# threewisemonkeys-as/torched_impala

Hardware: NVIDIA H100
Metric: learner steps/sec on synthetic (T=20,B=4096) trajectories (higher is better)
Workload: dtype f32

## Files before the change

torched_impala_b200/_cabi.py:

```python
from __future__ import annotations

import ctypes as C
import os

_HERE = os.path.dirname(os.path.abspath(__file__))
LIB_PATH = os.path.join(_HERE, "lib", "libimpala_b200.so")

MODE_REFERENCE = 0
MODE_PAPER = 1
MODES = {"reference": MODE_REFERENCE, "paper": MODE_PAPER}

OBS_F32 = 0
OBS_U8 = 1
OBS_DTYPES = {"float32": OBS_F32, "uint8": OBS_U8}

OPT_ADAM = 0
OPT_RMSPROP = 1
OPT_RULES = {"adam": OPT_ADAM, "rmsprop": OPT_RMSPROP}
POPART_STATS = 5
REWARD_CLIP_ABS_ONE = 1
REWARD_CLIP_SOFT_ASYMMETRIC = 2
REWARD_CLIPS = {"abs_one": REWARD_CLIP_ABS_ONE, "soft_asymmetric": REWARD_CLIP_SOFT_ASYMMETRIC}


def obs_dtype_code(obs_dtype: str) -> int:
    if obs_dtype not in OBS_DTYPES:
        raise ValueError(f"obs_dtype must be one of {sorted(OBS_DTYPES)}, got {obs_dtype!r}")
    return OBS_DTYPES[obs_dtype]


def reward_clip_code(reward_clip) -> int:
    if reward_clip is None:
        return 0
    if not isinstance(reward_clip, str) or reward_clip not in REWARD_CLIPS:
        raise ValueError(f"reward_clip must be None or one of {sorted(REWARD_CLIPS)}, got {reward_clip!r}")
    return REWARD_CLIPS[reward_clip]

ACT_CATEGORICAL = 0
ACT_GAUSSIAN = 1
ACT_DISTS = {"categorical": ACT_CATEGORICAL, "gaussian": ACT_GAUSSIAN}
MAX_GAUSSIAN_DIMS = 16


def act_kind_code(action_dist: str) -> int:
    if not isinstance(action_dist, str) or action_dist not in ACT_DISTS:
        raise ValueError(f"action_dist must be one of {sorted(ACT_DISTS)}, got {action_dist!r}")
    return ACT_DISTS[action_dist]


_ERRORS = {-1: "IMPALA_ERR_BAD_ARG", -2: "IMPALA_ERR_UNSUPPORTED_SHAPE",
           -3: "IMPALA_ERR_WORKSPACE_TOO_SMALL"}

_p = C.c_void_p
_i = C.c_int
_i64 = C.c_int64
_f = C.c_float

SIGNATURES = {
    "impala_abi_version": (_i, []),
# ... 113 lines not shown
```

torched_impala_b200/build.py:

```python
from __future__ import annotations

import concurrent.futures as cf
import os
import shutil
import subprocess
import sys

HERE = os.path.dirname(os.path.abspath(__file__))
CSRC = os.path.join(HERE, "csrc")
_LIB_DIR = os.environ.get("IMPALA_LIB_DIR", os.path.join(HERE, "lib"))
OBJ = os.path.join(_LIB_DIR, "obj")
LIB = os.path.join(_LIB_DIR, "libimpala_b200.so")

ARCH = ["-gencode", "arch=compute_90a,code=sm_90a"]
COMMON = ["-O3", "-lineinfo", "-std=c++17", "-Xcompiler", "-fPIC", "-Xptxas", "-v"]
MLP_WIDTHS = (8, 24, 32, 64, 128)


def _nvcc() -> str:
    for cand in (shutil.which("nvcc"), "/usr/local/cuda/bin/nvcc"):
        if cand and os.path.exists(cand):
            return cand
    raise RuntimeError("nvcc not found: the CUDA extension cannot be built")


def _units():
    units = [("mlp", "mlp.cu", []), ("vtrace_loss", "vtrace_loss.cu", []),
             ("vtrace_loss_rclip", "vtrace_loss_rclip.cu", []), ("vtrace_loss_gauss", "vtrace_loss_gauss.cu", []),
             ("optim", "optim.cu", []), ("abi", "abi.cu", []),
             ("mlp_fwd_tc", "mlp_fwd_tc.cu", []), ("mlp_bwd_tc", "mlp_bwd_tc.cu", []),
             ("loss_terms", "loss_terms.cu", []), ("mlp_obs_tc", "mlp_obs_tc.cu", []),
             ("obs_frames", "obs_frames.cu", []), ("batch_compose", "batch_compose.cu", [])]
    for op in MLP_WIDTHS:
        for bwd in (0, 1):
            units.append((f"mlp_inst_op{op}_{'bwd' if bwd else 'fwd'}", "mlp_inst.cu",
                          [f"-DIMPALA_OP={op}", f"-DIMPALA_BWD={bwd}"]))
    return units


def _newest_source_mtime() -> float:
    paths = [os.path.join(CSRC, f) for f in os.listdir(CSRC)]
    paths.append(os.path.join(HERE, "..", "include", "impala_b200.h"))
    paths.append(os.path.abspath(__file__))
    return max(os.path.getmtime(p) for p in paths)


def _compile(nvcc, name, src, defs, stamp):
    obj = os.path.join(OBJ, name + ".o")
    log = os.path.join(OBJ, name + ".ptxas.log")
    if os.path.exists(obj) and os.path.getmtime(obj) >= stamp:
        return name, 0, "cached"
    cmd = [nvcc, *ARCH, *COMMON, *defs, "-c", os.path.join(CSRC, src), "-o", obj]
    res = subprocess.run(cmd, capture_output=True, text=True)
    with open(log, "w") as f:
        f.write(res.stderr)
    return name, res.returncode, res.stderr if res.returncode else "built"


def build(verbose: bool = False, jobs: int | None = None) -> str:
    nvcc = _nvcc()
    os.makedirs(OBJ, exist_ok=True)
    stamp = _newest_source_mtime()
    units = _units()
    jobs = jobs or min(len(units), os.cpu_count() or 4)
    with cf.ThreadPoolExecutor(jobs) as ex:
        results = list(ex.map(lambda u: _compile(nvcc, *u, stamp), units))
    for name, rc, msg in results:
        if rc:
            raise RuntimeError(f"nvcc failed on {name}:\n{msg}")
        if verbose:
            print(f"[build] {name}: {msg}")
    objs = [os.path.join(OBJ, u[0] + ".o") for u in units]
    if (not os.path.exists(LIB)) or any(os.path.getmtime(o) > os.path.getmtime(LIB) for o in objs):
        cmd = [nvcc, *ARCH, "-shared", "-cudart", "static", "-o", LIB, *objs]
        res = subprocess.run(cmd, capture_output=True, text=True)
        if res.returncode:
            raise RuntimeError(f"link failed:\n{res.stderr}")
        if verbose:
            print(f"[build] linked {LIB}")
    return LIB


if __name__ == "__main__":
    print(build(verbose=True))
    sys.exit(0)
```

torched_impala_b200/csrc/mlp_bwd_tc.cu:

```cuda
#include "mlp_kernels.cuh"
#include "tc_common.cuh"

namespace {

constexpr int kRowsT = 64;
constexpr int kWG = 2;
constexpr int kThreads = kWG * 128;
constexpr int kWarps = kThreads / 32;
constexpr int kHB = 64 * kWG;
constexpr int kXAtomBytes = kRowsT * 128;

struct BwdTcArgs {
    const float* x;
    const float* params;
    const float* dout;
    float* ws;
    double* grad;
    unsigned int* ctl;
    int M, O, H, N2, num_tiles;
    MlpLayout lay;
};

struct BwdTcSplitArgs : BwdTcArgs {
    const float* dout_b;
    int M_a;
};
template <bool SPLIT>
using BwdArgs = std::conditional_t<SPLIT, BwdTcSplitArgs, BwdTcArgs>;

template <bool SPLIT>
__device__ __forceinline__ float load_dz(const BwdArgs<SPLIT>& a, int row, int n0, int n) {
    if constexpr (SPLIT) return split_dz(a.dout, a.dout_b, a.M_a, a.N2, row, n0 + n);
    else return __ldg(a.dout + (size_t)row * a.N2 + n0 + n);
}

__host__ __device__ constexpr size_t bwd_smem_bytes(int ka, int np) {
    return 1024 + (size_t)2 * ka * kHB * 128 + (size_t)2 * ka * (ka == 4 ? 32 : kRowsT) * 128 +
           (size_t)2 * ((ka == 4 ? 32 : kRowsT) / 32) * 32 * ka * 128 +
           (size_t)(ka == 4 ? 32 : kRowsT) * (np > 4 ? np + 4 : np) * sizeof(float) +
           (np > 4 ? (size_t)kHB * (np + 4) * sizeof(float) + 8 * 32 * sizeof(float) : 4 * sizeof(float));
}

__device__ __forceinline__ float f4(const float4& v, int e) { return e == 0 ? v.x : e == 1 ? v.y : e == 2 ? v.z : v.w; }

template <int NP, int KA, bool SPLIT = false>
__device__ __forceinline__ uint8_t* bwd_tc_body(const BwdArgs<SPLIT>& a, const int cta, const int ncta) {
    extern __shared__ uint8_t smem_raw[];
    uint8_t* smem = smem_raw + ((1024u - (tc::smem_u32(smem_raw) & 1023u)) & 1023u);
    constexpr bool X4 = KA == 4;
    constexpr bool L2S = NP > 4;
    constexpr int RT = X4 ? 32 : kRowsT;
    constexpr int NB = RT / 32;
    constexpr int FA = X4 ? 2 : KA;
// ... 438 lines not shown
        for (int sgm = 0; sgm < 4; ++sgm)
            for (int64_t p = lo4[sgm] + tid; p < hi4[sgm]; p += kThreads) wsb[p] = 0.f;
    }

    constexpr int kLd = kRowsT * 8 / 128;
    const int rr = 16 * warp + (lane & 15);
    float4 v[kLd];
    float z[NP];
    auto load = [&](int tile) {
#pragma unroll
        for (int k = 0; k < kLd; ++k) {
            const int c = 2 * k + (lane >> 4), row = tile * kRowsT + rr;
            v[k] = make_float4(0.f, 0.f, 0.f, 0.f);
            if (k < ksteps && tile < a.num_tiles && row < a.M && c < ochunks)
                v[k] = __ldg(reinterpret_cast<const float4*>(a.x + (size_t)row * O) + c);
        }
        const int row = tile * kRowsT + lt;
#pragma unroll
        for (int n = 0; n < NP; ++n)
            z[n] = (lt < kRowsT && tile < a.num_tiles && row < a.M && n < a.N2) ? load_dz<SPLIT>(a, row, 0, n) : 0.f;
    };
    float gb2[NP];
#pragma unroll
    for (int n = 0; n < NP; ++n) gb2[n] = 0.f;

    pdl_wait();
    const int j0 = 64 * grp + 16 * warp + g, j1 = j0 + 8;
    uint32_t wh[4][4], wl[4][4];
#pragma unroll
    for (int kk = 0; kk < 4; ++kk)
#pragma unroll
        for (int i = 0; i < 4; ++i) {
            const int f = 8 * kk + q + 4 * (i >> 1);
            float hi, lo;
            tc::split_tf32(f < O ? __ldg(W1 + (size_t)(i & 1 ? j1 : j0) * O + f) : 0.f, hi, lo);
            wh[kk][i] = __float_as_uint(hi), wl[kk][i] = __float_as_uint(lo);
        }
    const float bj0 = __ldg(b1 + j0), bj1 = __ldg(b1 + j1);
    float w2r0[NP], w2r1[NP], gw0[NP], gw1[NP], gb10 = 0.f, gb11 = 0.f;
#pragma unroll
    for (int n = 0; n < NP; ++n) {
        w2r0[n] = n < a.N2 ? __ldg(W2 + (size_t)n * H + j0) : 0.f;
        w2r1[n] = n < a.N2 ? __ldg(W2 + (size_t)n * H + j1) : 0.f;
        gw0[n] = gw1[n] = 0.f;
    }
    float acc_hh[16], acc_c[16];
#pragma unroll
    for (int i = 0; i < 16; ++i) acc_hh[i] = acc_c[i] = 0.f;
    tc::fence_acc(acc_hh), tc::fence_acc(acc_c);
    const uint64_t dx_hi = tc::smem_desc_k_sw128(x_hi, 0), dx_lo = tc::smem_desc_k_sw128(x_lo, 0);
    const uint64_t dxt_hi = tc::smem_desc_k_sw128(xt_hi, 0), dxt_lo = tc::smem_desc_k_sw128(xt_lo, 0);

    const int bar = 1 + wg, tstride = 2 * cpg;
    load(r + cpg * wg);
    for (int tile = r + cpg * wg; tile < a.num_tiles; tile += tstride) {
        tc::named_bar(bar, 128);
#pragma unroll
        for (int k = 0; k < kLd; ++k) {
            if (k >= ksteps) continue;
            const int c = 2 * k + (lane >> 4);
            float4 hi, lo;
            tc::split4(v[k], hi, lo);
            const uint32_t off = tc::sw128_offset(rr, c);
            *reinterpret_cast<float4*>(x_hi + off) = hi;
            *reinterpret_cast<float4*>(x_lo + off) = lo;
            const int r32 = rr & 31, pos = (r32 & ~7) + ((r32 & 7) >> 1) + 4 * (r32 & 1);
#pragma unroll
            for (int e = 0; e < 4; ++e) {
                const int f = 4 * c + e;
                const uint32_t toff = (rr >> 5) * (32 * 128) + (f >> 3) * 1024 + (f & 7) * 128 +
                                      (((pos >> 2) ^ (f & 7)) << 4) + (pos & 3) * 4;
                *reinterpret_cast<float*>(xt_hi + toff) = f4(hi, e);
                *reinterpret_cast<float*>(xt_lo + toff) = f4(lo, e);
            }
        }
        if (lt < kRowsT) {
#pragma unroll
            for (int n = 0; n < NP; ++n) dzs[lt * NP + n] = z[n], gb2[n] += z[n];
        }
        tc::fence_proxy_async();
        tc::named_bar(bar, 128);
        load(tile + tstride);

        uint64_t bx_hi = dx_hi, bx_lo = dx_lo;
        asm volatile("" : "+l"(bx_hi), "+l"(bx_lo));
        float d[32];
#pragma unroll
        for (int i = 0; i < 32; ++i) d[i] = 0.f;
        tc::fence_acc(d);
        tc::wgmma_fence();
#pragma unroll
        for (int kk = 0; kk < 4; ++kk) {
            if (kk < ksteps) {
                const uint32_t xo = (kk * 32) >> 4;
                tc::wgmma_n64_rs(d, wl[kk], bx_hi + xo, kk > 0);
                tc::wgmma_n64_rs(d, wh[kk], bx_lo + xo, true);
            }
        }
#pragma unroll
        for (int kk = 0; kk < 4; ++kk) {
            if (kk < ksteps) tc::wgmma_n64_rs(d, wh[kk], bx_hi + ((kk * 32) >> 4), true);
        }
        tc::wgmma_commit();
        tc::wgmma_wait<0>();
        tc::fence_acc(d);

#pragma unroll
        for (int i = 0; i < 8; ++i) {
#pragma unroll
            for (int e = 0; e < 2; ++e) {
                const int m = 8 * i + 2 * q + e;
                float dz[NP];
                if constexpr (NP == 4) {
                    const float4 t = *reinterpret_cast<const float4*>(dzs + 4 * m);
                    dz[0] = t.x, dz[1] = t.y, dz[2] = t.z, dz[3] = t.w;
                } else {
                    dz[0] = dzs[m];
                }
                const float pre0 = d[4 * i + e] + bj0, pre1 = d[4 * i + 2 + e] + bj1;
                const float h0 = fmaxf(pre0, 0.f), h1 = fmaxf(pre1, 0.f);
                float dh0 = dz[0] * w2r0[0], dh1 = dz[0] * w2r1[0];
#pragma unroll
                for (int n = 1; n < NP; ++n) dh0 = fmaf(dz[n], w2r0[n], dh0), dh1 = fmaf(dz[n], w2r1[n], dh1);
#pragma unroll
                for (int n = 0; n < NP; ++n) gw0[n] = fmaf(dz[n], h0, gw0[n]), gw1[n] = fmaf(dz[n], h1, gw1[n]);
                const float dp0 = pre0 > 0.f ? dh0 : 0.f, dp1 = pre1 > 0.f ? dh1 : 0.f;
                gb10 += dp0, gb11 += dp1;
                d[4 * i + e] = dp0, d[4 * i + 2 + e] = dp1;
            }
        }

        uint32_t lo[32];
#pragma unroll
        for (int i = 0; i < 32; ++i) {
            const float hi = __uint_as_float(__float_as_uint(d[i]) & 0xffffe000u);
            lo[i] = __float_as_uint(d[i] - hi);
            d[i] = hi;
        }
        uint64_t bxt_hi = dxt_hi, bxt_lo = dxt_lo;
        asm volatile("" : "+l"(bxt_hi), "+l"(bxt_lo));
        tc::wgmma_fence();
#pragma unroll
        for (int kk = 0; kk < 8; ++kk) {
            const uint32_t al[4] = {lo[4 * kk], lo[4 * kk + 2], lo[4 * kk + 1], lo[4 * kk + 3]};
            const uint32_t ah[4] = {__float_as_uint(d[4 * kk]), __float_as_uint(d[4 * kk + 2]),
                                    __float_as_uint(d[4 * kk + 1]), __float_as_uint(d[4 * kk + 3])};
            const uint32_t xo = ((kk >> 2) * 32 * 128 + (kk & 3) * 32) >> 4;
            tc::wgmma_n32_rs(acc_c, al, bxt_hi + xo, true);
            tc::wgmma_n32_rs(acc_c, ah, bxt_lo + xo, true);
            tc::wgmma_n32_rs(acc_hh, ah, bxt_hi + xo, true);
        }
        tc::wgmma_commit();
        tc::wgmma_wait<0>();
        tc::fence_acc(d);
#pragma unroll
        for (int i = 0; i < 32; ++i) asm volatile("" : "+r"(lo[i])::"memory");
        tc::fence_acc(acc_hh), tc::fence_acc(acc_c);
    }

#pragma unroll
    for (int s = 1; s <= 2; s <<= 1) {
        gb10 += __shfl_xor_sync(IMPALA_FULL_MASK, gb10, s);
        gb11 += __shfl_xor_sync(IMPALA_FULL_MASK, gb11, s);
#pragma unroll
        for (int n = 0; n < NP; ++n) {
            gw0[n] += __shfl_xor_sync(IMPALA_FULL_MASK, gw0[n], s);
            gw1[n] += __shfl_xor_sync(IMPALA_FULL_MASK, gw1[n], s);
        }
    }
    float gwt[16];
#pragma unroll
    for (int i = 0; i < 16; ++i) gwt[i] = acc_hh[i] + acc_c[i];
#pragma unroll
    for (int n = 0; n < NP; ++n) {
#pragma unroll
        for (int off = 16; off > 0; off >>= 1) gb2[n] += __shfl_xor_sync(IMPALA_FULL_MASK, gb2[n], off);
    }
    if (lt < kRowsT && lane == 0) {
#pragma unroll
        for (int n = 0; n < NP; ++n) gb2x[(2 * wg + warp) * 4 + n] = gb2[n];
    }
    float* xch = reinterpret_cast<float*>(smem + kStageBytes);
    __syncthreads();
    if (wg == 1) {
#pragma unroll
        for (int i = 0; i < 16; ++i) xch[i * 128 + lt] = gwt[i];
        xch[16 * 128 + lt] = gb10, xch[17 * 128 + lt] = gb11;
#pragma unroll
        for (int n = 0; n < NP; ++n) xch[(18 + n) * 128 + lt] = gw0[n], xch[(18 + NP + n) * 128 + lt] = gw1[n];
    }
    __syncthreads();
    if (wg == 0) {
#pragma unroll
        for (int i = 0; i < 16; ++i) gwt[i] += xch[i * 128 + lt];
        gb10 += xch[16 * 128 + lt], gb11 += xch[17 * 128 + lt];
#pragma unroll
        for (int n = 0; n < NP; ++n) gw0[n] += xch[(18 + n) * 128 + lt], gw1[n] += xch[(18 + NP + n) * 128 + lt];
        if (q == 0) {
            wsb[a.lay.ob1 + j0] = gb10;
            wsb[a.lay.ob1 + j1] = gb11;
#pragma unroll
            for (int n = 0; n < NP; ++n)
                if (n < a.N2) wsb[a.lay.oW2 + (size_t)n * H + j0] = gw0[n], wsb[a.lay.oW2 + (size_t)n * H + j1] = gw1[n];
        }
#pragma unroll
        for (int i = 0; i < 4; ++i) {
            const int f = 8 * i + 2 * q;
            if (f < O) {
                *reinterpret_cast<float2*>(wsb + a.lay.oW1 + (size_t)j0 * O + f) = make_float2(gwt[4 * i], gwt[4 * i + 1]);
                *reinterpret_cast<float2*>(wsb + a.lay.oW1 + (size_t)j1 * O + f) = make_float2(gwt[4 * i + 2], gwt[4 * i + 3]);
            }
        }
        if (grp == 0 && tid == 0) {
#pragma unroll
            for (int n = 0; n < NP; ++n)
                if (n < a.N2) wsb[a.lay.ob2 + n] = (gb2x[n] + gb2x[4 + n]) + (gb2x[8 + n] + gb2x[12 + n]);
        }
    }
    __threadfence();
    __syncthreads();
    return smem;
}

__device__ __forceinline__ void grid_arrive_and_wait(unsigned int* ctl) {
    if (threadIdx.x == 0) {
        atomicAdd(ctl, 1u);
        const long long t0 = clock64();
        unsigned int seen;
        do {
            asm volatile("ld.acquire.gpu.global.u32 %0, [%1];" : "=r"(seen) : "l"(ctl) : "memory");
            if (seen != gridDim.x && clock64() - t0 > (1ll << 32)) __trap();
        } while (seen != gridDim.x);
    }
    __syncthreads();
}

__device__ __forceinline__ void grid_depart(unsigned int* ctl) {
    if (threadIdx.x == 0 && atomicAdd(ctl + 1, 1u) == gridDim.x - 1) {
        ctl[0] = 0u;
        ctl[1] = 0u;
    }
}

__device__ __forceinline__ void reduce_rows(const BwdTcArgs& a, const int nparts, const int first,
                                            const int stride, double* s_red, const PushArgs* push = nullptr,
                                            const int64_t push_off = 0) {
    const int warp = threadIdx.x >> 5, lane = threadIdx.x & 31;
    const int64_t total = a.lay.total;
    const int nchunks = (int)((total + 63) >> 6);
    for (int c = first; c < nchunks; c += stride) {
        const int64_t e0 = (int64_t)c * 64 + 2 * lane;
        double sx = 0.0, sy = 0.0;
        if (e0 < total) {
            const float* col = a.ws + e0;
            int p = warp;
            for (; p + 3 * kWarps < nparts; p += 4 * kWarps) {
                const float2 v0 = __ldcg(reinterpret_cast<const float2*>(col + (size_t)p * total));
                const float2 v1 = __ldcg(reinterpret_cast<const float2*>(col + (size_t)(p + kWarps) * total));
                const float2 v2 = __ldcg(reinterpret_cast<const float2*>(col + (size_t)(p + 2 * kWarps) * total));
                const float2 v3 = __ldcg(reinterpret_cast<const float2*>(col + (size_t)(p + 3 * kWarps) * total));
                sx += v0.x, sy += v0.y, sx += v1.x, sy += v1.y;
                sx += v2.x, sy += v2.y, sx += v3.x, sy += v3.y;
            }
            for (; p < nparts; p += kWarps) {
                const float2 v0 = __ldcg(reinterpret_cast<const float2*>(col + (size_t)p * total));
                sx += v0.x, sy += v0.y;
            }
        }
        s_red[warp * 64 + 2 * lane] = sx;
        s_red[warp * 64 + 2 * lane + 1] = sy;
        __syncthreads();
        if (push) {
            if (warp < push->world) {
// ... 126 lines not shown
    if (cpg < 1) return IMPALA_ERR_UNSUPPORTED_SHAPE;
    e = dout_b ? impala_launch_ex(mlp_bwd_tc_split_kernel, nblk * cpg, kThreads, smem, st, true, true, a)
               : impala_launch_ex(kernel, nblk * cpg, kThreads, smem, st, true, true, static_cast<const BwdTcArgs&>(a));
    if (e != cudaSuccess) return (int)e;
    return impala_launch_status();
}

int impala_mlp_bwd_tc_pair(const float* x, const float* params_pi, const float* params_vf,
                           const float* dlogits, const float* dv, float* ws_pi, float* ws_vf,
                           double* grad_pi, double* grad_vf, unsigned int* ctl, int M_pi, int M_vf, int O,
                           int H_pi, int H_vf, int A, cudaStream_t st, const PushArgs* push, const double* extra,
                           int n_extra) {
    const BwdTcArgs a_pi = make_bwd_args(x, params_pi, dlogits, ws_pi, grad_pi, ctl, M_pi, O, H_pi, A);
    const BwdTcArgs a_vf = make_bwd_args(x, params_vf, dv, ws_vf, grad_vf, ctl, M_vf, O, H_vf, 1);
    const size_t smem = kBlkSmemBytes;
    cudaError_t e;
    int sms = 0;
    if ((e = impala_sm_count(&sms)) != cudaSuccess) return (int)e;
    int per_sm = 0;
    e = impala_resident_ctas(push ? (const void*)mlp_bwd_tc_pair_kernel<true> : (const void*)mlp_bwd_tc_pair_kernel<false>,
                             kThreads, smem, &per_sm);
    if (e != cudaSuccess) return (int)e;
    const int gp = H_pi / 64, gv = H_vf / 64;
    int grid = sms < kMaxParts ? sms : kMaxParts;
    if (grid < gp + gv) return IMPALA_ERR_UNSUPPORTED_SHAPE;
    int sp = 1, sv = 1;
    split_sets(a_pi.num_tiles, a_vf.num_tiles, grid, gp, gv, impala_env_int("IMPALA_PAIR_W_BWD", 125), 100, &sp, &sv);
    grid = gp * sp + gv * sv;
    const int n_pi = gp * sp;
    e = push ? impala_launch_ex(mlp_bwd_tc_pair_kernel<true>, grid, kThreads, smem, st, true, true, a_pi, a_vf, n_pi,
                                *push, extra, n_extra)
             : impala_launch_ex(mlp_bwd_tc_pair_kernel<false>, grid, kThreads, smem, st, true, true, a_pi, a_vf, n_pi,
                                PushArgs{}, (const double*)nullptr, 0);
    if (e != cudaSuccess) return (int)e;
    return impala_launch_status();
}

int impala_mlp_bwd_tcw(const MlpPlan& p, const float* x, const float* params, const float* dout, float* ws, int M,
                       int O, int H, int N2, cudaStream_t st, int* nparts, const float* dout_b, int M_a) {
    BwdTcSplitArgs a{make_bwd_args(x, params, dout, ws, nullptr, nullptr, M, O, H, N2), dout_b, M_a};
    a.num_tiles = (M + p.rows - 1) / p.rows;
    const int np = p.np;
    if (dout_b) {
        auto kernel = p.ka == 1   ? (np == 4 ? mlp_bwd_tcw_split_kernel<4, 1> : mlp_bwd_tcw_split_kernel<16, 1>)
                      : p.ka == 2 ? (np == 4 ? mlp_bwd_tcw_split_kernel<4, 2> : mlp_bwd_tcw_split_kernel<16, 2>)
                                  : (np == 4 ? mlp_bwd_tcw_split_kernel<4, 4> : mlp_bwd_tcw_split_kernel<32, 4>);
        return launch_tcw(kernel, p, a, st, nparts);
    }
    auto kernel = p.ka == 1   ? (np == 1 ? mlp_bwd_tcw_kernel<1, 1> : np == 4 ? mlp_bwd_tcw_kernel<4, 1> : mlp_bwd_tcw_kernel<16, 1>)
                  : p.ka == 2 ? (np == 1 ? mlp_bwd_tcw_kernel<1, 2> : np == 4 ? mlp_bwd_tcw_kernel<4, 2> : mlp_bwd_tcw_kernel<16, 2>)
                              : (np == 1 ? mlp_bwd_tcw_kernel<1, 4> : np == 4 ? mlp_bwd_tcw_kernel<4, 4> : mlp_bwd_tcw_kernel<32, 4>);
    return launch_tcw(kernel, p, static_cast<const BwdTcArgs&>(a), st, nparts);
}
```

torched_impala_b200/csrc/mlp_fwd_tc.cu:

```cuda
#include "mlp_fwd_tc.cuh"
#include "tc_common.cuh"

namespace {

constexpr int kWG = 2;
constexpr int kThreads = kWG * 128;
constexpr int kXAtomBytes = kTileM * 128;

__host__ __device__ constexpr bool x_in_regs(int ka) { return ka == 1; }

__host__ __device__ constexpr size_t fwd_smem_bytes(int hb, int ka, int np) {
    return 1024  + (size_t)2 * ka * hb * 128 +
           (x_in_regs(ka) ? 0 : (size_t)kWG * 2 * ka * kXAtomBytes) + (size_t)hb * (w2s_stride(np) + 1) * sizeof(float);
}

constexpr int kStageLd = 8;

template <int NP, int KA>
__device__ __forceinline__ void stage_weights(const FwdTcArgs& a, int p, uint8_t* w_hi, uint8_t* w_lo, float* b1s,
                                              float* w2s) {
    constexpr int NPS = w2s_stride(NP);
    const int HB = a.hb, ochunks = a.O >> 2, tid = threadIdx.x;
    const float* __restrict__ W1 = a.params + a.lay.oW1;
    const float* __restrict__ b1 = a.params + a.lay.ob1;
    const float* __restrict__ W2 = a.params + a.lay.oW2;
    const int n_w1 = HB * 8 * KA, n_w2 = HB * NP;
    for (int base = tid; base < n_w1; base += kStageLd * kThreads) {
        float4 w[kStageLd];
#pragma unroll
        for (int u = 0; u < kStageLd; ++u) {
            const int idx = base + u * kThreads, r = idx / (8 * KA), c = idx % (8 * KA);
            w[u] = make_float4(0.f, 0.f, 0.f, 0.f);
            if (idx < n_w1 && c < ochunks) w[u] = __ldg(reinterpret_cast<const float4*>(W1 + (size_t)(p * HB + r) * a.O) + c);
        }
#pragma unroll
        for (int u = 0; u < kStageLd; ++u) {
            const int idx = base + u * kThreads, r = idx / (8 * KA), c = idx % (8 * KA);
            if (idx < n_w1) {
                float4 hi, lo;
                tc::split4(w[u], hi, lo);
                const uint32_t off = (c >> 3) * (HB * 128) + tc::sw128_offset(r, c & 7);
                *reinterpret_cast<float4*>(w_hi + off) = hi;
                *reinterpret_cast<float4*>(w_lo + off) = lo;
            }
        }
    }
    for (int idx = tid; idx < HB; idx += kThreads) b1s[idx] = __ldg(b1 + p * HB + idx);
    for (int base = tid; base < n_w2; base += kStageLd * kThreads) {
        float w[kStageLd];
#pragma unroll
        for (int u = 0; u < kStageLd; ++u) {
            const int idx = base + u * kThreads, j = idx / NP, n = idx - j * NP;
            w[u] = idx < n_w2 && n < a.N2 ? __ldg(W2 + (size_t)n * a.H + p * HB + j) : 0.f;
        }
#pragma unroll
        for (int u = 0; u < kStageLd; ++u) {
            const int idx = base + u * kThreads, j = idx / NP, n = idx - j * NP;
            if (idx < n_w2) w2s[j * NPS + n] = w[u];
        }
    }
}

template <int NP, int KA, bool SPLIT = false>
__device__ __forceinline__ void fwd_rs_body(const FwdArgs<SPLIT>& a, const int cta, const int ncta) {
    extern __shared__ uint8_t smem_raw[];
    uint8_t* smem = smem_raw + ((1024u - (tc::smem_u32(smem_raw) & 1023u)) & 1023u);
    const int HB = a.hb;
    uint8_t* w_hi = smem;
    uint8_t* w_lo = w_hi + KA * HB * 128;
    float* b1s = reinterpret_cast<float*>(smem + 2 * KA * HB * 128);
    float* w2s = b1s + HB;
    const int tid = threadIdx.x, wg = tid >> 7, warp = (tid >> 5) & 3, lane = tid & 31;
    const int g = lane >> 2, q = lane & 3;
    const int O = a.O, ksteps = (O + 7) >> 3, nslices = HB / 32;
    const int unit = cta * kWG + wg, nunits = ncta * kWG;

    constexpr int KS = 4 * KA;
    float xr[KS][4];
    uint32_t xh[KS][4], xl[KS][4];
    auto load = [&](int tile) {
#pragma unroll
        for (int kk = 0; kk < KS; ++kk) {
#pragma unroll
            for (int i = 0; i < 4; ++i) {
                const int row = tile * kTileM + 16 * warp + g + 8 * (i & 1), f = 8 * kk + q + 4 * (i >> 1);
                xr[kk][i] = 0.f;
                if (kk < ksteps && tile < a.num_tiles && row < a.M && f < O) xr[kk][i] = __ldg(a.x + (size_t)row * O + f);
            }
        }
    };
    const uint64_t dw_hi = tc::smem_desc_k_sw128(w_hi, 0), dw_lo = tc::smem_desc_k_sw128(w_lo, 0);
    auto issue = [&](auto& d, int nc) {
        constexpr int ND = sizeof(d) / sizeof(float);
        auto mma = [&](const uint32_t(&x)[4], uint64_t bw, bool acc) {
            if constexpr (ND == 32) tc::wgmma_n64_rs(d, x, bw, acc);
            else tc::wgmma_n32_rs(d, x, bw, acc);
        };
        uint64_t bw_hi = dw_hi, bw_lo = dw_lo;
        asm volatile("" : "+l"(bw_hi), "+l"(bw_lo));
        auto wo = [&](int kk) -> uint32_t { return ((kk >> 2) * (HB * 128) + nc * 32 * 128 + (kk & 3) * 32) >> 4; };
#pragma unroll
        for (int i = 0; i < ND; ++i) d[i] = 0.f;
        tc::fence_acc(d);
        tc::wgmma_fence();
#pragma unroll
        for (int kk = 0; kk < KS; ++kk) {
            if (kk < ksteps) {
                mma(xl[kk], bw_hi + wo(kk), kk > 0);
                mma(xh[kk], bw_lo + wo(kk), true);
            }
        }
#pragma unroll
        for (int kk = 0; kk < KS; ++kk) {
            if (kk < ksteps) mma(xh[kk], bw_hi + wo(kk), true);
        }
        tc::wgmma_commit();
    };

    const int npass = a.H / HB;
    for (int p = 0; p < npass; ++p) {
        load(unit);
        __syncthreads();
        stage_weights<NP, KA>(a, p, w_hi, w_lo, b1s, w2s);
        tc::fence_proxy_async();
        __syncthreads();

        for (int tile = unit; tile < a.num_tiles; tile += nunits) {
#pragma unroll
            for (int kk = 0; kk < KS; ++kk) {
#pragma unroll
                for (int i = 0; i < 4; ++i) {
                    float hi, lo;
                    tc::split_tf32(xr[kk][i], hi, lo);
                    xh[kk][i] = __float_as_uint(hi), xl[kk][i] = __float_as_uint(lo);
                }
                tc::fence_frag(xh[kk]);
                tc::fence_frag(xl[kk]);
            }
            load(tile + nunits);

            float p0[NP], p1[NP];
#pragma unroll
            for (int n = 0; n < NP; ++n) p0[n] = 0.f, p1[n] = 0.f;
            int nc = 0;
            for (; nc + 2 <= nslices; nc += 2) {
                float d[32];
                issue(d, nc);
                tc::wgmma_wait<0>();
                tc::fence_acc(d);
                slice_epilogue<NP>(d, nc, q, b1s, w2s, p0, p1);
            }
            if (nc < nslices) {
                float d[16];
                issue(d, nc);
                tc::wgmma_wait<0>();
                tc::fence_acc(d);
                slice_epilogue<NP>(d, nc, q, b1s, w2s, p0, p1);
            }
            write_rows<NP, SPLIT>(a, p, tile, warp, g, q, p0, p1);
        }
    }
}

template <int NP, int KA, bool SPLIT = false>
__device__ __forceinline__ void fwd_ss_body(const FwdArgs<SPLIT>& a, const int cta, const int ncta) {
    extern __shared__ uint8_t smem_raw[];
    uint8_t* smem = smem_raw + ((1024u - (tc::smem_u32(smem_raw) & 1023u)) & 1023u);
    const int HB = a.hb;
    uint8_t* w_hi = smem;
    uint8_t* w_lo = w_hi + KA * HB * 128;
    const int tid = threadIdx.x, wg = tid >> 7, lt = tid & 127, warp = lt >> 5, lane = tid & 31;
    uint8_t* x_hi = w_lo + KA * HB * 128 + wg * 2 * KA * kXAtomBytes;
    uint8_t* x_lo = x_hi + KA * kXAtomBytes;
    float* b1s = reinterpret_cast<float*>(smem + 2 * KA * HB * 128 + kWG * 2 * KA * kXAtomBytes);
    float* w2s = b1s + HB;

    const int O = a.O, ochunks = O >> 2, ksteps = (O + 7) >> 3;
    const int unit = cta * kWG + wg, nunits = ncta * kWG;
    const int g = lane >> 2, q = lane & 3;

    constexpr int kLd = 4 * KA;
    float4 v[kLd];
    auto load = [&](int tile) {
#pragma unroll
        for (int k = 0; k < kLd; ++k) {
            const int idx = lt + 128 * k, r = idx / (8 * KA), c = idx % (8 * KA);
            const int row = tile * kTileM + r;
            v[k] = make_float4(0.f, 0.f, 0.f, 0.f);
            if (tile < a.num_tiles && row < a.M && c < ochunks)
                v[k] = __ldg(reinterpret_cast<const float4*>(a.x + (size_t)row * O) + c);
        }
    };

    const int npass = a.H / HB;
    for (int p = 0; p < npass; ++p) {
        load(unit);
        __syncthreads();
        stage_weights<NP, KA>(a, p, w_hi, w_lo, b1s, w2s);
        tc::fence_proxy_async();
        __syncthreads();

        for (int tile = unit; tile < a.num_tiles; tile += nunits) {
            tc::named_bar(1 + wg, 128);
#pragma unroll
            for (int k = 0; k < kLd; ++k) {
                const int idx = lt + 128 * k, r = idx / (8 * KA), c = idx % (8 * KA);
                float4 hi, lo;
                tc::split4(v[k], hi, lo);
                const uint32_t off = (c >> 3) * kXAtomBytes + tc::sw128_offset(r, c & 7);
                *reinterpret_cast<float4*>(x_hi + off) = hi;
                *reinterpret_cast<float4*>(x_lo + off) = lo;
            }
            tc::fence_proxy_async();
            tc::named_bar(1 + wg, 128);
// ... 81 lines not shown
}

template <int NP, int KA, bool SPLIT = false>
int launch_fwd(const FwdArgs<SPLIT>& a, cudaStream_t st) {
    const size_t smem = fwd_smem_bytes(a.hb, KA, NP);
    const void* kernel;
    if constexpr (SPLIT) kernel = (const void*)mlp_fwd_tc_split_kernel<NP, KA>;
    else kernel = (const void*)mlp_fwd_tc_kernel<NP, KA>;
    int grid = 0;
    const int rc = resident_grid(kernel, smem, &grid);
    if (rc != IMPALA_OK) return rc;
    const int want = (a.num_tiles + kWG - 1) / kWG;
    if constexpr (SPLIT) mlp_fwd_tc_split_kernel<NP, KA><<<want < grid ? want : grid, kThreads, smem, st>>>(a);
    else mlp_fwd_tc_kernel<NP, KA><<<want < grid ? want : grid, kThreads, smem, st>>>(a);
    return impala_launch_status();
}

template <int KA>
int launch_fwd_ka(int np, const FwdTcSplitArgs& a, cudaStream_t st) {
    if (a.out_b)
        return np == 4 ? launch_fwd<4, KA, true>(a, st) : np == 16 ? launch_fwd<16, KA, true>(a, st)
                                                        : launch_fwd<32, KA, true>(a, st);
    return np == 1 ? launch_fwd<1, KA>(a, st) : np == 4 ? launch_fwd<4, KA>(a, st)
                   : np == 16 ? launch_fwd<16, KA>(a, st) : launch_fwd<32, KA>(a, st);
}

}

int impala_mlp_fwd_tc(const MlpPlan& p, const float* x, const float* params, float* out, int M, int O, int H, int N2,
                      cudaStream_t st, float* out_b, int M_a) {
    const FwdTcSplitArgs a{make_fwd_args(x, params, out, M, O, H, N2, p.hb), out_b, M_a};
    return p.ka == 1 ? launch_fwd_ka<1>(p.np, a, st) : p.ka == 2 ? launch_fwd_ka<2>(p.np, a, st)
                                                     : launch_fwd_ka<4>(p.np, a, st);
}

int impala_mlp_fwd_tc_pair(const float* x, const float* params_pi, const float* params_vf, float* logits,
                           float* values, int M_pi, int M_vf, int O, int H_pi, int H_vf, int A,
                           cudaStream_t st) {
    const FwdTcArgs a_pi = make_fwd_args(x, params_pi, logits, M_pi, O, H_pi, A, H_pi);
    const FwdTcArgs a_vf = make_fwd_args(x, params_vf, values, M_vf, O, H_vf, 1, H_vf);
    const size_t s_pi = fwd_smem_bytes(a_pi.hb, 1, 4), s_vf = fwd_smem_bytes(a_vf.hb, 1, 4);
    const size_t smem = s_pi > s_vf ? s_pi : s_vf;
    int grid = 0;
    const int rc = resident_grid((const void*)mlp_fwd_tc_pair_kernel, smem, &grid);
    if (rc != IMPALA_OK) return rc;
    const int units_pi = (a_pi.num_tiles + kWG - 1) / kWG, units_vf = (a_vf.num_tiles + kWG - 1) / kWG;
    if (grid > units_pi + units_vf) grid = units_pi + units_vf;
    const int n_pi = impala_pair_split(units_pi, units_vf, grid,
                                       impala_env_int("IMPALA_PAIR_W_FWD", 100) * (H_pi / 32),
                                       100 * (H_vf / 32));
    mlp_fwd_tc_pair_kernel<<<grid, kThreads, smem, st>>>(a_pi, a_vf, n_pi);
    return impala_launch_status();
}
```

torched_impala_b200/csrc/tc_common.cuh:

```cuda
#pragma once

#include <cuda_runtime.h>
#include <stdint.h>

namespace tc {

__device__ __forceinline__ uint32_t smem_u32(const void* p) {
    return static_cast<uint32_t>(__cvta_generic_to_shared(p));
}

__device__ __forceinline__ void fence_proxy_async() {
    asm volatile("fence.proxy.async.shared::cta;" ::: "memory");
}

__device__ __forceinline__ void named_bar(int id, int nthreads) {
    asm volatile("bar.sync %0, %1;" ::"r"(id), "r"(nthreads) : "memory");
}

__device__ __forceinline__ uint64_t smem_desc_k_sw128(const void* tile, uint32_t byte_off) {
    const uint32_t addr = smem_u32(tile) + byte_off;
    uint64_t d = 0;
    d |= static_cast<uint64_t>((addr >> 4) & 0x3fff);
    d |= static_cast<uint64_t>(1) << 16;
    d |= static_cast<uint64_t>(1024 >> 4) << 32;
    d |= static_cast<uint64_t>(1) << 62;
    return d;
}

__device__ __forceinline__ void wgmma_fence() { asm volatile("wgmma.fence.sync.aligned;" ::: "memory"); }
__device__ __forceinline__ void wgmma_commit() { asm volatile("wgmma.commit_group.sync.aligned;" ::: "memory"); }
template <int N>
__device__ __forceinline__ void wgmma_wait() {
    asm volatile("wgmma.wait_group.sync.aligned %0;" ::"n"(N) : "memory");
}
template <int N>
__device__ __forceinline__ void fence_acc(float (&d)[N]) {
#pragma unroll
    for (int i = 0; i < N; ++i) asm volatile("" : "+f"(d[i])::"memory");
}
__device__ __forceinline__ void fence_frag(uint32_t (&a)[4]) {
#pragma unroll
    for (int i = 0; i < 4; ++i) asm volatile("" : "+r"(a[i])::"memory");
}

#define IMPALA_WG_D16                                                                                   \
    "{%0, %1, %2, %3, %4, %5, %6, %7, %8, %9, %10, %11, %12, %13, %14, %15}"
#define IMPALA_WG_D16_OPS(d)                                                                            \
    "+f"(d[0]), "+f"(d[1]), "+f"(d[2]), "+f"(d[3]), "+f"(d[4]), "+f"(d[5]), "+f"(d[6]), "+f"(d[7]),     \
        "+f"(d[8]), "+f"(d[9]), "+f"(d[10]), "+f"(d[11]), "+f"(d[12]), "+f"(d[13]), "+f"(d[14]),        \
        "+f"(d[15])

__device__ __forceinline__ void wgmma_n32_ss(float (&d)[16], uint64_t a_desc, uint64_t b_desc, bool accumulate) {
    asm volatile(
        "{\n\t"
        ".reg .pred p;\n\t"
        "setp.ne.b32 p, %18, 0;\n\t"
        "wgmma.mma_async.sync.aligned.m64n32k8.f32.tf32.tf32 " IMPALA_WG_D16 ", %16, %17, p, 1, 1;\n\t"
        "}\n"
        : IMPALA_WG_D16_OPS(d)
        : "l"(a_desc), "l"(b_desc), "r"(accumulate ? 1 : 0));
}
__device__ __forceinline__ void wgmma_n32_rs(float (&d)[16], const uint32_t (&a)[4], uint64_t b_desc,
                                             bool accumulate) {
    asm volatile(
        "{\n\t"
        ".reg .pred p;\n\t"
        "setp.ne.b32 p, %21, 0;\n\t"
        "wgmma.mma_async.sync.aligned.m64n32k8.f32.tf32.tf32 " IMPALA_WG_D16 ", {%16, %17, %18, %19}, %20, p, 1, 1;\n\t"
        "}\n"
// ... 47 lines not shown
```

Baseline: 7253.

## Alternate GEMM turns between warpgroups via named barriers and add phase-clock profiling

Both the forward and backward tensor-core MLP kernels now pass a GEMM 'turn' between their two warpgroups using named bar.sync/bar.arrive pairs, so the warpgroups' wgmma issues alternate and each one's epilogue overlaps the other's GEMM. The backward kernel also moves the next tile's load to after the wgmma commit so it overlaps the in-flight GEMM. Optional compile-time phase-clock instrumentation is added but is off by default. The turn-taking adds barrier waits and tail-balancing logic that could serialize work or deadlock if the tile counts are handled wrongly.

```diff
diff --git a/torched_impala_b200/_cabi.py b/torched_impala_b200/_cabi.py
--- a/torched_impala_b200/_cabi.py
+++ b/torched_impala_b200/_cabi.py
@@ -4,7 +4,7 @@
 import os
 
 _HERE = os.path.dirname(os.path.abspath(__file__))
-LIB_PATH = os.path.join(_HERE, "lib", "libimpala_b200.so")
+LIB_PATH = os.path.join(os.environ.get("IMPALA_LIB_DIR", os.path.join(_HERE, "lib")), "libimpala_b200.so")
 
 MODE_REFERENCE = 0
 MODE_PAPER = 1
diff --git a/torched_impala_b200/build.py b/torched_impala_b200/build.py
--- a/torched_impala_b200/build.py
+++ b/torched_impala_b200/build.py
@@ -9,6 +9,7 @@
 HERE = os.path.dirname(os.path.abspath(__file__))
 CSRC = os.path.join(HERE, "csrc")
 _LIB_DIR = os.environ.get("IMPALA_LIB_DIR", os.path.join(HERE, "lib"))
+_DEFS = ["-DIMPALA_PHASE_CLOCKS"] if os.environ.get("IMPALA_PHASE_CLOCKS") == "1" else []
 OBJ = os.path.join(_LIB_DIR, "obj")
 LIB = os.path.join(_LIB_DIR, "libimpala_b200.so")
 
@@ -50,7 +51,7 @@
     log = os.path.join(OBJ, name + ".ptxas.log")
     if os.path.exists(obj) and os.path.getmtime(obj) >= stamp:
         return name, 0, "cached"
-    cmd = [nvcc, *ARCH, *COMMON, *defs, "-c", os.path.join(CSRC, src), "-o", obj]
+    cmd = [nvcc, *ARCH, *COMMON, *_DEFS, *defs, "-c", os.path.join(CSRC, src), "-o", obj]
     res = subprocess.run(cmd, capture_output=True, text=True)
     with open(log, "w") as f:
         f.write(res.stderr)
@@ -61,6 +62,13 @@
     nvcc = _nvcc()
     os.makedirs(OBJ, exist_ok=True)
     stamp = _newest_source_mtime()
+    defs_file = os.path.join(OBJ, "defines.txt")
+    defs = " ".join(_DEFS)
+    built_with = open(defs_file).read() if os.path.exists(defs_file) else None
+    if built_with != defs:
+        stamp = float("inf")
+        if built_with is not None:
+            os.remove(defs_file)
     units = _units()
     jobs = jobs or min(len(units), os.cpu_count() or 4)
     with cf.ThreadPoolExecutor(jobs) as ex:
@@ -70,6 +78,8 @@
             raise RuntimeError(f"nvcc failed on {name}:\n{msg}")
         if verbose:
             print(f"[build] {name}: {msg}")
+    with open(defs_file, "w") as f:
+        f.write(defs)
     objs = [os.path.join(OBJ, u[0] + ".o") for u in units]
     if (not os.path.exists(LIB)) or any(os.path.getmtime(o) > os.path.getmtime(LIB) for o in objs):
         cmd = [nvcc, *ARCH, "-shared", "-cudart", "static", "-o", LIB, *objs]
diff --git a/torched_impala_b200/csrc/mlp_bwd_tc.cu b/torched_impala_b200/csrc/mlp_bwd_tc.cu
--- a/torched_impala_b200/csrc/mlp_bwd_tc.cu
+++ b/torched_impala_b200/csrc/mlp_bwd_tc.cu
@@ -1,4 +1,5 @@
 #include "mlp_kernels.cuh"
+#include "phase_clocks.cuh"
 #include "tc_common.cuh"
 
 namespace {
@@ -543,9 +544,13 @@
     const uint64_t dxt_hi = tc::smem_desc_k_sw128(xt_hi, 0), dxt_lo = tc::smem_desc_k_sw128(xt_lo, 0);
 
     const int bar = 1 + wg, tstride = 2 * cpg;
+    const int own = 3 + wg, other = 4 - wg;
+    PHASE_BEGIN(wg);
     load(r + cpg * wg);
     for (int tile = r + cpg * wg; tile < a.num_tiles; tile += tstride) {
+        PHASE_TILE(wg);
         tc::named_bar(bar, 128);
+        PHASE_MARK(wg, 0);
 #pragma unroll
         for (int k = 0; k < kLd; ++k) {
             if (k >= ksteps) continue;
@@ -571,7 +576,7 @@
         }
         tc::fence_proxy_async();
         tc::named_bar(bar, 128);
-        load(tile + tstride);
+        PHASE_MARK(wg, 1);
 
         uint64_t bx_hi = dx_hi, bx_lo = dx_lo;
         asm volatile("" : "+l"(bx_hi), "+l"(bx_lo));
@@ -579,6 +584,7 @@
 #pragma unroll
         for (int i = 0; i < 32; ++i) d[i] = 0.f;
         tc::fence_acc(d);
+        PHASE_GEMM_ON(wg);
         tc::wgmma_fence();
 #pragma unroll
         for (int kk = 0; kk < 4; ++kk) {
@@ -593,8 +599,11 @@
             if (kk < ksteps) tc::wgmma_n64_rs(d, wh[kk], bx_hi + ((kk * 32) >> 4), true);
         }
         tc::wgmma_commit();
+        load(tile + tstride);
         tc::wgmma_wait<0>();
         tc::fence_acc(d);
+        PHASE_GEMM_OFF(wg);
+        PHASE_MARK(wg, 2);
 
 #pragma unroll
         for (int i = 0; i < 8; ++i) {
@@ -630,6 +639,10 @@
         }
         uint64_t bxt_hi = dxt_hi, bxt_lo = dxt_lo;
         asm volatile("" : "+l"(bxt_hi), "+l"(bxt_lo));
+        PHASE_MARK(wg, 3);
+        tc::named_bar_if(wg == 1 || tile != r, own, 256);
+        PHASE_MARK(wg, 5);
+        PHASE_GEMM_ON(wg);
         tc::wgmma_fence();
 #pragma unroll
         for (int kk = 0; kk < 8; ++kk) {
@@ -642,11 +655,17 @@
             tc::wgmma_n32_rs(acc_hh, ah, bxt_hi + xo, true);
         }
         tc::wgmma_commit();
+        tc::named_bar_arrive_if(wg == 0 || tile + cpg < a.num_tiles, other, 256);
         tc::wgmma_wait<0>();
         tc::fence_acc(d);
 #pragma unroll
         for (int i = 0; i < 32; ++i) asm volatile("" : "+r"(lo[i])::"memory");
         tc::fence_acc(acc_hh), tc::fence_acc(acc_c);
+        PHASE_GEMM_OFF(wg);
+        PHASE_MARK(wg, 4);
+    }
+    if (wg == 1 && (r < a.num_tiles ? (a.num_tiles - 1 - r) / cpg + 1 : 0) % 2 == 1) {
+        tc::named_bar(own, 256);
     }
 
 #pragma unroll
@@ -710,6 +729,7 @@
     }
     __threadfence();
     __syncthreads();
+    PHASE_END(wg);
     return smem;
 }
 
@@ -942,3 +962,12 @@
                               : (np == 1 ? mlp_bwd_tcw_kernel<1, 4> : np == 4 ? mlp_bwd_tcw_kernel<4, 4> : mlp_bwd_tcw_kernel<32, 4>);
     return launch_tcw(kernel, p, static_cast<const BwdTcArgs&>(a), st, nparts);
 }
+
+#ifdef IMPALA_PHASE_CLOCKS
+IMPALA_PHASE_READER(impala_phase_read_bwd)
+
+extern "C" int impala_phase_read(unsigned long long* out, int reset) {
+    const int e = impala_phase_read_bwd(out, reset);
+    return e ? e : impala_phase_read_fwd(out + phase::kSlots, reset);
+}
+#endif
diff --git a/torched_impala_b200/csrc/mlp_fwd_tc.cu b/torched_impala_b200/csrc/mlp_fwd_tc.cu
--- a/torched_impala_b200/csrc/mlp_fwd_tc.cu
+++ b/torched_impala_b200/csrc/mlp_fwd_tc.cu
@@ -1,4 +1,5 @@
 #include "mlp_fwd_tc.cuh"
+#include "phase_clocks.cuh"
 #include "tc_common.cuh"
 
 namespace {
@@ -70,7 +71,8 @@
     uint8_t* w_lo = w_hi + KA * HB * 128;
     float* b1s = reinterpret_cast<float*>(smem + 2 * KA * HB * 128);
     float* w2s = b1s + HB;
-    const int tid = threadIdx.x, wg = tid >> 7, warp = (tid >> 5) & 3, lane = tid & 31;
+    const int wg = __shfl_sync(IMPALA_FULL_MASK, (int)threadIdx.x >> 7, 0);
+    const int tid = threadIdx.x, warp = (tid >> 5) & 3, lane = tid & 31;
     const int g = lane >> 2, q = lane & 3;
     const int O = a.O, ksteps = (O + 7) >> 3, nslices = HB / 32;
     const int unit = cta * kWG + wg, nunits = ncta * kWG;
@@ -117,6 +119,12 @@
         tc::wgmma_commit();
     };
 
+    const int nb = (nslices + 1) / 2;
+    auto turn = [&](bool first) { tc::named_bar_if(wg == 1 || !first, 3 + wg, 256); };
+    auto pass_turn = [&](bool last, int tile) {
+        tc::named_bar_arrive_if(wg == 0 || !last || tile - 1 + nunits < a.num_tiles, 4 - wg, 256);
+    };
+    PHASE_BEGIN(wg);
     const int npass = a.H / HB;
     for (int p = 0; p < npass; ++p) {
         load(unit);
@@ -124,8 +132,11 @@
         stage_weights<NP, KA>(a, p, w_hi, w_lo, b1s, w2s);
         tc::fence_proxy_async();
         __syncthreads();
-
-        for (int tile = unit; tile < a.num_tiles; tile += nunits) {
+        PHASE_MARK(wg, 5);
+
+        int tile = unit;
+        for (; tile < a.num_tiles; tile += nunits) {
+            PHASE_TILE(wg);
 #pragma unroll
             for (int kk = 0; kk < KS; ++kk) {
 #pragma unroll
@@ -138,6 +149,7 @@
                 tc::fence_frag(xl[kk]);
             }
             load(tile + nunits);
+            PHASE_MARK(wg, 2);
 
             float p0[NP], p1[NP];
 #pragma unroll
@@ -145,21 +157,44 @@
             int nc = 0;
             for (; nc + 2 <= nslices; nc += 2) {
                 float d[32];
+                turn(tile == unit && nc == 0);
+                PHASE_MARK(wg, 4);
+                PHASE_GEMM_ON(wg);
                 issue(d, nc);
+                pass_turn(nc + 2 >= nslices, tile);
                 tc::wgmma_wait<0>();
                 tc::fence_acc(d);
+                PHASE_GEMM_OFF(wg);
+                PHASE_MARK(wg, 0);
                 slice_epilogue<NP>(d, nc, q, b1s, w2s, p0, p1);
+                PHASE_MARK(wg, 1);
             }
             if (nc < nslices) {
                 float d[16];
+                turn(tile == unit && nc == 0);
+                PHASE_MARK(wg, 4);
+                PHASE_GEMM_ON(wg);
                 issue(d, nc);
+                pass_turn(true, tile);
                 tc::wgmma_wait<0>();
                 tc::fence_acc(d);
+                PHASE_GEMM_OFF(wg);
+                PHASE_MARK(wg, 0);
                 slice_epilogue<NP>(d, nc, q, b1s, w2s, p0, p1);
+                PHASE_MARK(wg, 1);
             }
             write_rows<NP, SPLIT>(a, p, tile, warp, g, q, p0, p1);
+            PHASE_MARK(wg, 3);
+        }
+        if (wg == 1 && tile - 1 < a.num_tiles) {
+            for (int b = 0; b < nb; ++b) {
+                tc::named_bar(4, 256);
+                if (b + 1 < nb) tc::named_bar_arrive(3, 256);
+            }
         }
     }
+    PHASE_SYNC();
+    PHASE_END(wg);
 }
 
 template <int NP, int KA, bool SPLIT = false>
@@ -347,3 +382,7 @@
     mlp_fwd_tc_pair_kernel<<<grid, kThreads, smem, st>>>(a_pi, a_vf, n_pi);
     return impala_launch_status();
 }
+
+#ifdef IMPALA_PHASE_CLOCKS
+IMPALA_PHASE_READER(impala_phase_read_fwd)
+#endif
diff --git a/torched_impala_b200/csrc/phase_clocks.cuh b/torched_impala_b200/csrc/phase_clocks.cuh
--- /dev/null
+++ b/torched_impala_b200/csrc/phase_clocks.cuh
@@ -0,0 +1,97 @@
+#pragma once
+
+#include <stdint.h>
+
+namespace phase {
+constexpr int kPhases = 8;
+enum : int {
+    kTiles = kPhases,
+    kOverlap,
+    kWindows,
+    kWgCycles,
+    kCtaNs,
+    kCtas,
+    kFirstNs,
+    kLastNs,
+    kSlots
+};
+}
+
+#ifdef IMPALA_PHASE_CLOCKS
+
+namespace phase {
+__device__ __forceinline__ unsigned long long globaltimer() {
+    unsigned long long t;
+    asm volatile("mov.u64 %0, %%globaltimer;" : "=l"(t));
+    return t;
+}
+}
+
+static __device__ unsigned long long impala_phase_buf[phase::kSlots];
+
+#define PHASE_BEGIN(wg)                                                                                     \
+    __shared__ unsigned long long pc_s[2][16];                                                              \
+    __shared__ unsigned long long pc_ns0;                                                                   \
+    const bool pc_on = (threadIdx.x & 127) == 0;                                                            \
+    if (threadIdx.x < 32) pc_s[threadIdx.x >> 4][threadIdx.x & 15] = 0ull;                                  \
+    __syncthreads();                                                                                        \
+    if (pc_on) {                                                                                            \
+        pc_s[wg][11] = pc_s[wg][12] = (unsigned long long)clock64();                                        \
+        if (threadIdx.x == 0) pc_ns0 = phase::globaltimer();                                                \
+    }
+#define PHASE_MARK(wg, k)                                                                                   \
+    if (pc_on) {                                                                                            \
+        const unsigned long long t_ = (unsigned long long)clock64();                                        \
+        pc_s[wg][k] += t_ - pc_s[wg][11];                                                                   \
+        pc_s[wg][11] = t_;                                                                                  \
+    }
+#define PHASE_GEMM_ON(wg)                                                                                   \
+    if (pc_on) {                                                                                            \
+        pc_s[wg][10] += 1ull;                                                                               \
+        pc_s[wg][9] += *(volatile unsigned long long*)&pc_s[(wg) ^ 1][13] != 0ull;                          \
+        *(volatile unsigned long long*)&pc_s[wg][13] = 1ull;                                                \
+    }
+#define PHASE_GEMM_OFF(wg)                                                                                  \
+    if (pc_on) *(volatile unsigned long long*)&pc_s[wg][13] = 0ull;
+#define PHASE_TILE(wg)                                                                                      \
+    if (pc_on) pc_s[wg][8] += 1ull;
+#define PHASE_SYNC() __syncthreads()
+#define PHASE_END(wg)                                                                                       \
+    if (pc_on) {                                                                                            \
+        for (int i_ = 0; i_ < phase::kPhases; ++i_) atomicAdd(&impala_phase_buf[i_], pc_s[wg][i_]);         \
+        atomicAdd(&impala_phase_buf[phase::kTiles], pc_s[wg][8]);                                           \
+        atomicAdd(&impala_phase_buf[phase::kOverlap], pc_s[wg][9]);                                         \
+        atomicAdd(&impala_phase_buf[phase::kWindows], pc_s[wg][10]);                                        \
+        atomicAdd(&impala_phase_buf[phase::kWgCycles], (unsigned long long)clock64() - pc_s[wg][12]);       \
+        if (threadIdx.x == 0) {                                                                             \
+            const unsigned long long e_ = phase::globaltimer();                                             \
+            atomicAdd(&impala_phase_buf[phase::kCtaNs], e_ - pc_ns0);                                       \
+            atomicAdd(&impala_phase_buf[phase::kCtas], 1ull);                                               \
+            atomicMin(&impala_phase_buf[phase::kFirstNs], pc_ns0);                                          \
+            atomicMax(&impala_phase_buf[phase::kLastNs], e_);                                               \
+        }                                                                                                   \
+    }
+#define IMPALA_PHASE_READER(name)                                                                           \
+    int name(unsigned long long* out, int reset) {                                                          \
+        if (cudaMemcpyFromSymbol(out, impala_phase_buf, sizeof(impala_phase_buf)) != cudaSuccess) return -1; \
+        if (reset) {                                                                                        \
+            unsigned long long z[phase::kSlots] = {};                                                       \
+            z[phase::kFirstNs] = ~0ull;                                                                     \
+            if (cudaMemcpyToSymbol(impala_phase_buf, z, sizeof(z)) != cudaSuccess) return -1;               \
+        }                                                                                                   \
+        return 0;                                                                                           \
+    }
+int impala_phase_read_bwd(unsigned long long* out, int reset);
+int impala_phase_read_fwd(unsigned long long* out, int reset);
+
+#else
+
+#define PHASE_BEGIN(wg)
+#define PHASE_MARK(wg, k)
+#define PHASE_GEMM_ON(wg)
+#define PHASE_GEMM_OFF(wg)
+#define PHASE_TILE(wg)
+#define PHASE_SYNC()
+#define PHASE_END(wg)
+
+#endif
diff --git a/torched_impala_b200/csrc/tc_common.cuh b/torched_impala_b200/csrc/tc_common.cuh
--- a/torched_impala_b200/csrc/tc_common.cuh
+++ b/torched_impala_b200/csrc/tc_common.cuh
@@ -15,6 +15,17 @@
 
 __device__ __forceinline__ void named_bar(int id, int nthreads) {
     asm volatile("bar.sync %0, %1;" ::"r"(id), "r"(nthreads) : "memory");
+}
+__device__ __forceinline__ void named_bar_arrive(int id, int nthreads) {
+    asm volatile("bar.arrive %0, %1;" ::"r"(id), "r"(nthreads) : "memory");
+}
+__device__ __forceinline__ void named_bar_if(bool pred, int id, int nthreads) {
+    asm volatile("{\n\t.reg .pred p;\n\tsetp.ne.b32 p, %2, 0;\n\t@p bar.sync %0, %1;\n\t}" ::"r"(id), "r"(nthreads),
+                 "r"((int)pred) : "memory");
+}
+__device__ __forceinline__ void named_bar_arrive_if(bool pred, int id, int nthreads) {
+    asm volatile("{\n\t.reg .pred p;\n\tsetp.ne.b32 p, %2, 0;\n\t@p bar.arrive %0, %1;\n\t}" ::"r"(id), "r"(nthreads),
+                 "r"((int)pred) : "memory");
 }
 
 __device__ __forceinline__ uint64_t smem_desc_k_sw128(const void* tile, uint32_t byte_off) {
```

Result: faster. 7949 (median of 6 runs) (+9.6%).
